# jing2li/MGPreconditionedGCR

Measured on AMD Instinct MI355X. Metric: gcr_iterations_per_sec, higher is better.
Workload: dtype f64; 1 GPU; 3D 7-point Poisson 128^3 per GPU, unpreconditioned GCR restart 5, complex fp64, x0=0, RHS splitmix64 seed 0; rows=2097152, nnz=14581760, complex=True, stored_matrix_bytes=2097292, ell_width=7, tail_nnz=0, partition=1 GPU

## Files before the change

mgpreconditionedgcr_amd/csrc/api.hip:

```cpp
#include <algorithm>
#include <numeric>

#include <cstring>

#include "internal.h"

using namespace mgcr;

#define LOCK() std::lock_guard<std::recursive_mutex> lk__(ctx().mtx)

extern "C" {

int mgcr_csr_create(int64_t nrow, int64_t ncol, const int64_t *rowptr, const int64_t *col, const double *val_ri,
                    mgcr_op_t *out) {
    MGCR_TRY(require_ctx());
    MGCR_CHECK(out && rowptr && (col || rowptr[nrow] == 0) && (val_ri || rowptr[nrow] == 0), MGCR_ERR_INVALID,
               "mgcr_csr_create: null argument");
    LOCK();
    mgcr_op_s *op = new mgcr_op_s();
    op->kind = OP_CSR;
    op->dim = ncol;
    op->nrow = nrow;
    int rc = csr_build_device(nrow, ncol, rowptr, col, val_ri, &op->csr);
    if (rc != MGCR_OK) { delete op; return rc; }
// ... 191 lines not shown

int mgcr_op_halo_kind(mgcr_op_t op, int32_t *kind) {
    MGCR_CHECK(op && kind, MGCR_ERR_INVALID, "mgcr_op_halo_kind: null argument");
    MGCR_REFUSE_EVENODD_MULTI(op, "mgcr_op_halo_kind");
    MGCR_REFUSE_GCR32(op, "mgcr_op_halo_kind");
    const Op *o = op_matrix(op);
    MGCR_CHECK(o->dist, MGCR_ERR_UNSUPPORTED, "mgcr_op_halo_kind: not a distributed Sparse");
    *kind = dist_halo_kind(o->dist);
    return MGCR_OK;
}

int mgcr_set_option(const char *name, int value, int *previous) {
    MGCR_CHECK(name, MGCR_ERR_INVALID, "null option name");
    if (!strcmp(name, "spmv_part")) {
        const int p = set_spmv_part(value);
        if (previous) *previous = p;
        return MGCR_OK;
    }
    bool prev;
    if (!strcmp(name, "pattern_storage")) prev = set_patterns_enabled(value != 0);
    else if (!strcmp(name, "stencil_storage")) prev = set_stencil_enabled(value != 0);
    else if (!strcmp(name, "lean_cycles")) prev = set_lean_enabled(value != 0);
    else if (!strcmp(name, "fused_apply")) prev = set_fuse_enabled(value != 0);
    else if (!strcmp(name, "graph_replay")) prev = set_graph_enabled(value != 0);
    else if (!strcmp(name, "resident_solver")) prev = set_resident_enabled(value != 0);
    else if (!strcmp(name, "step_build")) prev = set_stepbuild_enabled(value != 0);
    else if (!strcmp(name, "start_build")) prev = set_start_build_enabled(value != 0);
    else if (!strcmp(name, "step_build_keep_r")) {
        static bool last = true;
        prev = last;
        last = value != 0;
    }
    else if (!strcmp(name, "step_build_keep_all")) prev = set_stepbuild_keep_all_enabled(value != 0);
    else if (!strcmp(name, "halo_split")) prev = set_halo_split(value != 0);
    else if (!strcmp(name, "pw_tail")) prev = set_pw_tail_enabled(value != 0);
    else { set_error("mgcr_set_option: unknown option '%s'", name); return MGCR_ERR_INVALID; }
    if (previous) *previous = prev ? 1 : 0;
    return MGCR_OK;
}

int mgcr_stat(const char *name, int64_t *value) {
    MGCR_CHECK(name && value, MGCR_ERR_INVALID, "mgcr_stat: null argument");
    if (!strcmp(name, "resident_solves")) *value = resident_solve_count();
    else if (!strcmp(name, "step_build_launches")) *value = stepbuild_launch_count();
    else if (!strcmp(name, "step_keep_wide_launches")) *value = stepbuild_keep_wide_launch_count();
    else if (!strcmp(name, "step_apply_own_launches")) *value = stepbuild_apply_own_launch_count();
    else if (!strcmp(name, "start_build_launches")) *value = start_build_launch_count();
    else if (!strcmp(name, "small_solves")) *value = gcr_small_solve_count();
    else if (!strcmp(name, "one_launch_fallbacks")) *value = gcr_fallback_count();
    else if (!strcmp(name, "halo_split_exchanges")) *value = dist_halo_split_count();
    else if (!strcmp(name, "pw_tail_folds")) *value = comm_pw_tail_count();
    else if (!strcmp(name, "multi_solves")) *value = gcr_multi_solve_count();
    else if (!strcmp(name, "queue_solves")) *value = gcr_queue_stat(0);
    else if (!strcmp(name, "queue_admissions")) *value = gcr_queue_stat(1);
    else if (!strcmp(name, "queue_steps")) *value = gcr_queue_stat(2);
    else if (!strcmp(name, "eo_queue_solves")) *value = gcr_queue_stat(3);
    else if (!strcmp(name, "eo_queue_admissions")) *value = gcr_queue_stat(4);
    else if (!strcmp(name, "eo_queue_steps")) *value = gcr_queue_stat(5);
    else if (!strcmp(name, "evenodd_fused_steps")) *value = eo_fused_step_count();
    else if (!strcmp(name, "evenodd_diag_fused_steps")) *value = eo_diag_fused_step_count();
    else if (!strcmp(name, "evenodd_block_applies")) *value = eo_block_apply_count();
    else if (!strcmp(name, "evenodd_block_fused_steps")) *value = eo_block_fused_step_count();
    else if (!strcmp(name, "gcr32_applies")) *value = gcr32_apply_count();
    else if (!strcmp(name, "gcr32_steps")) *value = gcr32_step_count();
    else { set_error("mgcr_stat: unknown counter '%s'", name); return MGCR_ERR_INVALID; }
    return MGCR_OK;
}

int mgcr_selftest_coherence(int32_t steps, int32_t coherent, int64_t *rows_wrong) {
    MGCR_TRY(require_ctx());
    LOCK();
    return coherence_selftest(steps, coherent, rows_wrong);
}

int mgcr_op_stored_bytes(mgcr_op_t op, int64_t *matrix_bytes, int32_t *ell_width, int64_t *tail_nnz) {
    MGCR_CHECK(op, MGCR_ERR_INVALID, "null operator");
    MGCR_REFUSE_EVENODD_MULTI(op, "mgcr_op_stored_bytes");
    MGCR_REFUSE_GCR32(op, "mgcr_op_stored_bytes");
    const Op *o = op_matrix(op);
// ... 283 lines not shown
```

mgpreconditionedgcr_amd/csrc/gcr_stepbuild.hip:

```cpp
#include <climits>
#include <cstdlib>
#include <type_traits>

#include "internal.h"
#include "reduce.h"
#include "gcr_dev.h"
#include "spmv_dev.h"
#include "exchange_dev.h"

namespace mgcr {

constexpr int SB_MAX_TRIPS = 4;
constexpr int SB_MAX_ND = 5;
constexpr int SB_KEEP_TB = 2;
#ifndef MGCR_SB_KEEP_MORE
#define MGCR_SB_KEEP_MORE 1
#endif
template <bool WIDE, int NDT, bool XR, bool CLOSE, bool REALC> constexpr int sb_kept_rows() {
    if (NDT == 1) return 3;
    if (!REALC || !MGCR_SB_KEEP_MORE) return WIDE ? 0 : 2;
    if (!WIDE) return !XR && CLOSE ? 4 : 3;
    if (NDT == 4) return CLOSE ? 4 : 1;
    return XR ? 2 : 3;
}
#ifndef MGCR_SB_TEMPORAL_TAIL
#define MGCR_SB_TEMPORAL_TAIL -1
#endif
template <bool WIDE, int NDT, bool XR, bool CLOSE, bool REALC> constexpr bool sb_temporal_tail() {
    if (MGCR_SB_TEMPORAL_TAIL >= 0) return MGCR_SB_TEMPORAL_TAIL != 0;
    return REALC && XR && (WIDE ? (NDT == 4 && !CLOSE) || (NDT == 5 && CLOSE) : NDT == 1 && !CLOSE);
}
template <int TB_, int KT_, bool OTF_, int APPLY_, bool TAIL_> struct SbKeepPolicy {
    static constexpr int TB = TB_, KT = KT_;
    static constexpr bool OTF = OTF_, TAIL = TAIL_;
    static constexpr bool OWN = APPLY_ >= 1, LANES = APPLY_ >= 2;
};
#ifndef MGCR_SB_APPLY
#define MGCR_SB_APPLY 1
#endif
template <bool WIDE, int NDT, bool XR, bool CLOSE, bool REALC> constexpr int sb_apply_form() { return REALC ? MGCR_SB_APPLY : 0; }
template <int NDT, bool XR, bool CLOSE> constexpr bool sb_close_merged() { return CLOSE && (NDT == 4 || (NDT == 5 && XR)); }

struct StepBuildArgs {
    RowMat m;
    const cplx *x;
    const cplx *aps[SB_MAX_ND];
    int64_t n;
    int nlogical;
    RowMap rm;
    DevState *st;
    int it;
    const double *partsR;
    int nblkR, strideR;
    double *hist;
    int hist_cap;
    const cplx *den;
    cplx *ap_out;
    double *partsA;
    LeanCoef *lc;
    const cplx *ps[SB_MAX_ND];
    cplx *p_out;
    cplx *xvec;
    cplx *xr_out;
    cplx *xr_den_slot;
    int xr_slot;
    double *partsR_out;
    v4i *slots;
    unsigned gen0;
    unsigned *abort_dev;
    int *abort_host;
    int spin_limit;
    int test_stall;
};

__device__ __forceinline__ cplx sb_xr_alpha(const ResSync &sy, DevState *st, LeanCoef *lc, cplx *xr_den_slot, int xr_slot, int lb) {
    const cplx num = make_double2(res_total(sy, 0), res_total(sy, 1)), den = make_double2(res_total(sy, 2), res_total(sy, 3));
    const cplx alpha = to_sgpr(cdiv(num, den));
    if (lb == 0 && threadIdx.x == 0) {
        *xr_den_slot = den;
        st->npend = xr_slot + 1;
    }
    if (lb == 0 && (int)threadIdx.x < LND) lean_pending_update(lc, xr_slot, alpha, (int)threadIdx.x);
    return alpha;
}

template <int MODE, int WT, int NDT, bool XR, bool CLOSE, bool REALC = false>
__global__ void __launch_bounds__(RED_THREADS, 8) step_build_kernel(StepBuildArgs a) {
    __shared__ double lds[(2 * NDT > 4 ? 2 * NDT : 4) * 17];
    __shared__ double lds_pw[2 * SB_MAX_ND * 17], lds_ws[2 * SB_MAX_ND * RES_GRP];
    __shared__ int gave_up;
    __shared__ cplx sbeta[NDT], scp[NDT];
    extern __shared__ __attribute__((aligned(16))) unsigned char sb_smem[];
    if (a.st->stop_at < a.st->base + a.it) return;
    const int lb = logical_workgroup(a.rm, (int)blockIdx.x, (int)gridDim.x);
    if (lb >= a.nlogical) return;
    cplx *arL = reinterpret_cast<cplx *>(sb_smem);
    ResSync sy;
    res_sync_init(sy, a.slots, a.gen0, a.nlogical, lb, a.abort_dev, a.spin_limit, lds_pw, lds_ws, &gave_up);
    if (a.test_stall && lb == a.test_stall - 1) return;
    int64_t i0, end, stride;
    row_range(a.rm, lb, a.nlogical, a.n, &i0, &end, &stride);
    {
        double v[2 * NDT];
#pragma unroll
        for (int j = 0; j < 2 * NDT; j++) v[j] = 0.;
        int trip = 0;
        for (int64_t i = i0; i < end; i += stride, trip++) {
            const PatLds pl{nullptr, nullptr, nullptr};
            cplx sum;
            if constexpr (REALC) sum = sten_row_product_t<WT, false, 1>(a.m, i, [&](int32_t j) -> cplx { return a.x[j]; });
            else sum = fused_row_product<MODE, WT>(a.m, i, 0, pl, [&](int32_t j) -> cplx { return a.x[j]; });
            const cplx yi = a.m.shift ? csub(a.x[i], cmul(a.m.k, sum)) : sum;
            arL[trip * RED_THREADS + (int)threadIdx.x] = yi;
            __builtin_amdgcn_sched_barrier(0);
            cplx b[NDT];
#pragma unroll
            for (int j = 0; j < NDT; j++) b[j] = ld_stream<true>(a.aps[j] + i);
// ... 124 lines not shown
    if (threadIdx.x < 4) a.partsA[threadIdx.x * RED_MAX_BLOCKS + lb] = mine;
    auto close_last = [&]() {
        if (trip > 0) {
            const int64_t il = i0 + (int64_t)(trip - 1) * stride;
            close_row(il, a.x[il]);
        }
        __builtin_amdgcn_sched_barrier(0);
    };
    if constexpr (XR) {
        if ((int)threadIdx.x < 4) {
            const v4i w4 = {__double2loint(mine), __double2hiint(mine), (int)sy.gen, 0};
            __builtin_amdgcn_raw_buffer_store_b128(w4, sy.slots, ((2 * RES_NV + (int)threadIdx.x) * RES_BLK + lb) * 16, 0, RES_SC1);
        }
        if constexpr (MERGED) close_last();
        const cplx xr0 = i0 < end ? a.x[i0] : make_double2(0., 0.);
        if (!res_collect<4>(sy, 2)) {
            res_abort(a.abort_dev, a.abort_host);
            for (int64_t i = i0; i < end; i += stride) a.xr_out[i] = make_double2(__builtin_nan(""), __builtin_nan(""));
            if (threadIdx.x == 0) a.partsR_out[lb] = __builtin_nan("");
            return;
        }
        if (ends_here) return;
        const cplx alpha = sb_xr_alpha(sy, a.st, a.lc, a.xr_den_slot, a.xr_slot, lb);
        double vr[1] = {0.};
        trip = 0;
        for (int64_t i = i0; i < end; i += stride, trip++) {
            const cplx rn = csub(i == i0 ? xr0 : a.x[i], cmul(alpha, arL[trip * RED_THREADS + (int)threadIdx.x]));
            a.xr_out[i] = rn;
            vr[0] += rn.x * rn.x + rn.y * rn.y;
        }
        const double tot = block_sum_owner<1>(vr, lds);
        if (threadIdx.x == 0) a.partsR_out[lb] = tot;
    }
}

template <class T>
__device__ __forceinline__ T *sb_elem(T *p, uint32_t off) {
    using C = std::conditional_t<std::is_const_v<T>, const char, char>;
    return reinterpret_cast<T *>(reinterpret_cast<C *>(p) + off);
}

__device__ __forceinline__ void sb_wave_pair_to_lds(double (&v)[2], double *lds, int k0) {
    double s;
    const int k = wave_multi_sum<2>(v, s);
    if (((int)threadIdx.x & 31) == 0) lds[(k0 + k) * 17 + ((int)threadIdx.x >> 6)] = s;
}
template <int NV>
__device__ __forceinline__ double sb_block_owner_from_lds(double *lds) {
    const int nwave = (blockDim.x + 63) >> 6;
    __syncthreads();
    double t = 0.;
    if (threadIdx.x < NV)
        for (int w = 0; w < nwave; w++) t += lds[threadIdx.x * 17 + w];
    return t;
}

template <int NDT>
__device__ __forceinline__ const cplx *sb_stage_src(const cplx *den, const LeanCoef *lc, int i) {
    if (i < NDT) return den + i;
    if (i < 2 * NDT) return lc->cx + (i - NDT);
    const int m = (i - 2 * NDT) / NDT, j = (i - 2 * NDT) % NDT;
    return m == 0 ? lc->t + j : lc->T + j * LND + m;
}
template <int NDT>
__device__ __forceinline__ cplx sb_stage_close_coef(const cplx *col, const cplx *sbeta, int m) {
    cplx c = make_double2(0., 0.);
    for (int j = m; j < NDT; j++) c = cadd(c, cmul(sbeta[j], j == m ? make_double2(1., 0.) : col[j]));
    return c;
}
__device__ __forceinline__ void sb_stage_rr_waves(double v, int nblk, double *lds_rr) {
    if (nblk == 1) {
        if (threadIdx.x == 0) lds_rr[16] = v;
        return;
    }
    double w[1] = {v}, s;
    wave_multi_sum<1>(w, s);
    if ((threadIdx.x & 63) == 0) lds_rr[threadIdx.x >> 6] = s;
}
__device__ __forceinline__ double sb_stage_rr(int nblk, const double *lds_rr) {
    if (nblk == 1) return lds_rr[16];
    const int nwave = (blockDim.x + 63) >> 6;
    double t = 0.;
    for (int w = 0; w < nwave; w++) t += lds_rr[w];
    return t;
}

template <int NDT, bool XR, bool CLOSE, bool REALC>
__global__ void __launch_bounds__(RED_THREADS, 8) step_keep_kernel(StepBuildArgs a) {
    using POL = SbKeepPolicy<SB_KEEP_TB, sb_kept_rows<false, NDT, XR, CLOSE, REALC>(), false, sb_apply_form<false, NDT, XR, CLOSE, REALC>(),
                             sb_temporal_tail<false, NDT, XR, CLOSE, REALC>()>;
#include "gcr_stepbuild_keep_body.h"
}
template <int NDT, bool XR, bool CLOSE, bool REALC>
__global__ void __launch_bounds__(RED_THREADS, 8) step_keep_wide_kernel(StepBuildArgs a) {
    using POL = SbKeepPolicy<1, sb_kept_rows<true, NDT, XR, CLOSE, REALC>(), NDT == 5 && XR, sb_apply_form<true, NDT, XR, CLOSE, REALC>(),
                             sb_temporal_tail<true, NDT, XR, CLOSE, REALC>()>;
#include "gcr_stepbuild_keep_body.h"
}

struct StartArgs {
    RowMat m;
    const cplx *b;
    cplx *ap0;
    int64_t n;
    int nlogical;
    RowMap rm;
    DevState *st;
    double *hist;
    LeanCoef *lc;
    cplx *den0;
    cplx *r_out;
    double *partsR_out;
    v4i *slots;
    unsigned gen0;
    unsigned *abort_dev;
    int *abort_host;
    int spin_limit;
// ... 54 lines not shown
        const double nb = res_total(sy, 4);
        a.st->bnorm2 = nb;
        a.st->rr = nb;
        a.hist[0] = sqrt(nb) / sqrt(nb);
    }
    const cplx alpha = sb_xr_alpha(sy, a.st, a.lc, a.den0, 0, lb);
    double vr[1] = {0.};
#pragma unroll
    for (int t = 0; t < SB_MAX_TRIPS; t++) {
        const int64_t i = i0 + (int64_t)t * stride;
        if (i < end) {
            const cplx rn = csub(t == 0 ? b0 : a.b[i], cmul(alpha, apL[t * RED_THREADS + (int)threadIdx.x]));
            a.r_out[i] = rn;
            vr[0] += rn.x * rn.x + rn.y * rn.y;
        }
    }
    const double tot = block_sum_owner<1>(vr, lds);
    if (threadIdx.x == 0) a.partsR_out[lb] = tot;
}

static EnvSwitch g_stepbuild{"MGCR_STEPBUILD"}, g_start_build{"MGCR_START_BUILD"};
static EnvSwitch g_sb_keep_all{"MGCR_SB_KEEP_ALL"};
static EnvSwitch g_sb_real{"MGCR_SB_REAL"};
bool stepbuild_is_enabled() { return g_stepbuild.on(); }
bool set_stepbuild_enabled(bool on) { return g_stepbuild.set(on); }
bool set_start_build_enabled(bool on) { return g_start_build.set(on); }
bool set_stepbuild_keep_all_enabled(bool on) { return g_sb_keep_all.set(on); }
static int64_t g_stepbuild_launches = 0;
int64_t stepbuild_launch_count() { return g_stepbuild_launches; }
static int64_t g_keep_wide_launches = 0;
int64_t stepbuild_keep_wide_launch_count() { return g_keep_wide_launches; }
static int64_t g_apply_own_launches = 0;
int64_t stepbuild_apply_own_launch_count() { return g_apply_own_launches; }

template <int NDT, bool XR, bool CLOSE> constexpr bool sb_keep_fits() { return NDT <= 2 || (NDT == 3 && !(XR && CLOSE)); }
template <int NDT, bool XR, bool CLOSE, bool R> const void *sb_keep(int *form) {
    *form = sb_apply_form<false, NDT, XR, CLOSE, R>();
    if constexpr (sb_keep_fits<NDT, XR, CLOSE>()) return (const void *)step_keep_kernel<NDT, XR, CLOSE, R>;
    else return nullptr;
}
template <int NDT, bool XR, bool CLOSE> constexpr bool sb_keep_wide_fits() { return (NDT == 4 && XR) || (NDT == 5 && CLOSE); }
template <int NDT, bool XR, bool CLOSE, bool R> const void *sb_keep_wide_form(int *form) {
    *form = sb_apply_form<true, NDT, XR, CLOSE, R>();
    if constexpr (sb_keep_wide_fits<NDT, XR, CLOSE>()) return (const void *)step_keep_wide_kernel<NDT, XR, CLOSE, R>;
    else return nullptr;
}
static const void *sb_keep_wide(int nd, bool xr, bool close, bool realc, int *form) {
#define SKR(NDT, R) (close ? (xr ? sb_keep_wide_form<NDT, true, true, R>(form) : sb_keep_wide_form<NDT, false, true, R>(form)) \
                           : (xr ? sb_keep_wide_form<NDT, true, false, R>(form) : sb_keep_wide_form<NDT, false, false, R>(form)))
#define SKK(NDT) (realc ? SKR(NDT, true) : SKR(NDT, false))
    return nd == 4 ? SKK(4) : nd == 5 ? SKK(5) : nullptr;
#undef SKK
#undef SKR
}
static const void *sb_kernel(int nd, bool xr, bool close, bool realc, bool mid, bool *wide = nullptr, bool *own = nullptr) {
    if (wide) *wide = false;
    if (own) *own = false;
    const void *keep = nullptr;
    int form = 0;
    if (g_sb_keep_all.on() && nd > 3) keep = sb_keep_wide(nd, xr, close, realc, &form);
    if (g_sb_keep_all.on() && nd <= 3) {
#define SKR(NDT, R) (close ? (xr ? sb_keep<NDT, true, true, R>(&form) : sb_keep<NDT, false, true, R>(&form)) \
                           : (xr ? sb_keep<NDT, true, false, R>(&form) : sb_keep<NDT, false, false, R>(&form)))
#define SKK(NDT) (realc ? SKR(NDT, true) : SKR(NDT, false))
        keep = nd == 1 ? SKK(1) : nd == 2 ? SKK(2) : SKK(3);
#undef SKK
// ... 66 lines not shown
    a.rm = rm;
    a.st = st;
    a.slots = sh.slots; a.abort_dev = sh.abort_dev; a.abort_host = sh.abort_host;
    a.gen0 = exchange_take_generations(ngen);
    a.test_stall = getenv("MGCR_TEST_STEPBUILD_STALL") ? atoi(getenv("MGCR_TEST_STEPBUILD_STALL")) : 0;
    a.spin_limit = getenv("MGCR_TEST_RESIDENT_SPIN_LIMIT") ? atoi(getenv("MGCR_TEST_RESIDENT_SPIN_LIMIT")) : RES_SPIN_LIMIT;
    return MGCR_OK;
}
static int sb_launch(const void *kernel, void *args, int grid, size_t lds_bytes, const char *who) {
    MGCR_CHECK(launch_is_coresident(kernel, RED_THREADS, lds_bytes, grid), MGCR_ERR_INVALID, "%s: launch would not be co-resident", who);
    void *kargs[1] = {args};
    MGCR_HIP(hipLaunchKernel(kernel, dim3((unsigned)grid), dim3(RED_THREADS), kargs, lds_bytes, ctx().stream));
    MGCR_HIP(hipGetLastError());
    return MGCR_OK;
}

int csr_step_build(const CsrDev &A, const cplx *x, bool shift, cplx k, const cplx *const *aps, int nd, DevState *st, int it, const double *partsR,
                   int nblkR, int strideR, double *hist, int hist_cap, const cplx *den, cplx *ap_out, double *partsA, LeanCoef *lc,
                   const RowMap &rm, cplx *xr_out, cplx *xr_den_slot, int xr_slot, double *partsR_out, const cplx *const *close_ps, cplx *close_p_out,
                   cplx *close_x) {
    MGCR_CHECK(nd >= 1 && nd <= SB_MAX_ND, MGCR_ERR_INVALID, "csr_step_build: 1..5 directions");
    StepBuildArgs a;
    MGCR_TRY(sb_fill_common(a, A, shift, k, st, rm, 3));
    a.x = x;
    for (int j = 0; j < SB_MAX_ND; j++) a.aps[j] = aps[j < nd ? j : 0];
    a.it = it; a.partsR = partsR; a.nblkR = nblkR; a.strideR = strideR; a.hist = hist; a.hist_cap = hist_cap;
    a.den = den; a.ap_out = ap_out; a.partsA = partsA; a.lc = lc;
    for (int j = 0; j < SB_MAX_ND; j++) a.ps[j] = close_ps ? close_ps[j < nd ? j : 0] : nullptr;
    a.p_out = close_p_out; a.xvec = close_x;
    a.xr_out = xr_out; a.xr_den_slot = xr_den_slot; a.xr_slot = xr_slot; a.partsR_out = partsR_out;
    const bool xr = xr_out != nullptr, close = close_ps != nullptr, realc = g_sb_real.on() && a.m.realv;
    bool wide, own;
    const void *kernel = sb_kernel(nd, xr, close, realc, sten_lane_middle(A), &wide, &own);
    MGCR_TRY(sb_launch(kernel, &a, a.nlogical, sb_lds_bytes(A, a.nlogical), "csr_step_build"));
    g_stepbuild_launches++;
    if (wide) g_keep_wide_launches++;
    if (own) g_apply_own_launches++;
    return MGCR_OK;
}

static int64_t g_start_build_launches = 0;
int64_t start_build_launch_count() { return g_start_build_launches; }
static const void *start_kernel(bool realc) {
    return realc ? (const void *)start_build_kernel<true> : (const void *)start_build_kernel<false>;
}

bool csr_start_build_eligible(const CsrDev &A, const DistCsr *dist) {
    if (!g_start_build.on() || !csr_step_build_eligible(A, dist, 1)) return false;
    const bool realc = g_sb_real.on() && row_mat(A, false, cplx{0., 0.}).realv;
    return launch_is_coresident(start_kernel(realc), RED_THREADS, sb_lds_bytes(A, red_grid(A.nrow)), red_grid(A.nrow));
}

int csr_start_build(const CsrDev &A, const cplx *b, bool shift, cplx k, cplx *ap0, DevState *st, double *hist, LeanCoef *lc, cplx *den0,
                    cplx *r_out, double *partsR_out, const RowMap &rm) {
    StartArgs a;
    MGCR_TRY(sb_fill_common(a, A, shift, k, st, rm, 1));
    a.b = b;
    a.ap0 = ap0;
    a.hist = hist; a.lc = lc; a.den0 = den0; a.r_out = r_out; a.partsR_out = partsR_out;
    MGCR_TRY(sb_launch(start_kernel(g_sb_real.on() && a.m.realv), &a, a.nlogical, sb_lds_bytes(A, a.nlogical), "csr_start_build"));
    g_start_build_launches++;
    return MGCR_OK;
}

}
```

mgpreconditionedgcr_amd/csrc/internal.h:

```cpp
#pragma once
#include <hip/hip_runtime.h>
#include <climits>
#include <cstdint>
#include <cstdio>
#include <cstdlib>
#include <cstring>
#include <mutex>
#include <string>
#include <type_traits>
#include <utility>
#include <vector>

#include "../../include/mgcr.h"

namespace mgcr {

typedef double2 cplx;

void set_error(const char *fmt, ...);
int hip_fail(hipError_t e, const char *what, const char *file, int line);

#define MGCR_HIP(call)                                                     \
    do {                                                                   \
        hipError_t e__ = (call);                                           \
// ... 204 lines not shown
template <typename F>
static int dispatch_bool(bool b, F &&f) { return b ? f(std::true_type{}) : f(std::false_type{}); }
template <typename... KA, typename... AA>
static int launch(void (*kernel)(KA...), unsigned grid, int block, size_t lds, AA... args) {
    hipLaunchKernelGGL(kernel, dim3(grid), dim3(block), lds, ctx().stream, args...);
    MGCR_HIP(hipGetLastError());
    return MGCR_OK;
}

int csr_build_device(int64_t nrow, int64_t ncol, const int64_t *h_rowptr, const int64_t *h_col,
                     const double *h_val_ri, CsrDev *out);
void csr_free(CsrDev *c);
bool set_patterns_enabled(bool on);
bool set_stencil_enabled(bool on);
bool stencil_enabled();
int ell_band_count(const CsrDev &A, unsigned long long *d_cnt);
bool csr_stencil_active(const CsrDev &A);
int set_spmv_part(int part);
bool set_lean_enabled(bool on);
bool set_fuse_enabled(bool on);
bool set_graph_enabled(bool on);
bool set_resident_enabled(bool on);
constexpr int MGCR_INT_GAVE_UP = 1001;
int resident_check(bool internal = false);
void resident_shutdown();
int64_t resident_solve_count();
bool set_stepbuild_enabled(bool on);
int64_t stepbuild_launch_count();
int64_t stepbuild_keep_wide_launch_count();
int64_t stepbuild_apply_own_launch_count();
bool set_start_build_enabled(bool on);
int64_t start_build_launch_count();
bool set_stepbuild_keep_all_enabled(bool on);
int coherence_selftest(int steps, int coherent, int64_t *rows_wrong);
bool stepbuild_is_enabled();
bool launch_is_coresident(const void *kernel, int threads, size_t dyn_lds, int grid);
bool one_launch_paths_enabled();
int csr_apply(const CsrDev &A, const cplx *x, cplx *y, bool shift, cplx k, DistCsr *dist = nullptr, const cplx *w = nullptr);
bool csr_fusable(const CsrDev &A, const DistCsr *dist);
bool fuse_enabled();
struct RowMap;
struct PwTail;
bool csr_step_apply_has_pw_tail(const CsrDev &A, const DistCsr *dist);
int csr_step_apply(const CsrDev &A, const cplx *x, cplx *y, bool shift, cplx k, const cplx *const *vecs, int nd, double *parts,
                   DistCsr *dist, const RowMap &rm, const PwTail *pw = nullptr);
struct DevState;
struct LeanCoef;
bool csr_xr_fusable(const CsrDev &A, const DistCsr *dist);
bool csr_apply_carry(const CsrDev &A, const cplx *x, cplx *y, bool shift, cplx k, const cplx *w);
int csr_xr_fuse_kind(const CsrDev &A, const DistCsr *dist);
int csr_step_apply_xr(const CsrDev &A, const cplx *r_in, const cplx *ap, cplx *r_out, cplx *y, bool shift, cplx k, const cplx *const *vecs,
                      int nd, double *parts, double *partsR, DevState *st, int it, const double *partsA, int nblkA, int strideA,
                      cplx *den_slot, int slot, LeanCoef *lc, const RowMap &rm);
int csr_init_apply(const CsrDev &A, const cplx *r0, cplx *aps0, bool shift, cplx k, const cplx *b, double *partsA, double *partsR,
                   double *partsN, DistCsr *dist, const RowMap &rm);
int bcsr_build_device(int32_t nbrow, int32_t nbcol, int32_t bs, const int32_t *h_browptr, const int32_t *h_bcol,
                      const double *h_blocks, BcsrDev *out);
void bcsr_free(BcsrDev *b);
int bcsr_apply(const BcsrDev &A, const cplx *x, cplx *y, const cplx *xh = nullptr, int32_t nb_own = INT32_MAX);

struct SkipRef {
    const int *p = nullptr;
    int it = 0;
};
void set_apply_skip(SkipRef s);
SkipRef get_apply_skip();
// ... 121 lines not shown
```

Measured before the change: 16200 it/s.

## Add paired-workgroup step-build kernel merging two logical blocks per CTA

Adds a new step_pair_kernel in which each physical workgroup handles two logical workgroups, launched on half the grid (256 instead of 512) when the logical grid is 512 and the kernel can be co-resident. Each thread keeps more rows of Ap_0/Ap_1 in registers, and one combined poll/collect serves both logical blocks. The aim is to cut the cost of grid-wide synchronisation and to reuse more data held on chip in the fused GCR step. The cost is higher register pressure (launch bounds lowered to 4) and fewer resident waves. It applies only to realc, xr, non-shifted forms with keep_all on, and is gated by the MGCR_SB_PAIR env switch, whose default is not visible.

Result: faster. 16860 it/s (median of 6 runs) (+4.0%).

```diff
diff --git a/mgpreconditionedgcr_amd/csrc/api.hip b/mgpreconditionedgcr_amd/csrc/api.hip
--- a/mgpreconditionedgcr_amd/csrc/api.hip
+++ b/mgpreconditionedgcr_amd/csrc/api.hip
@@ -247,6 +247,7 @@
         last = value != 0;
     }
     else if (!strcmp(name, "step_build_keep_all")) prev = set_stepbuild_keep_all_enabled(value != 0);
+    else if (!strcmp(name, "step_build_pair")) prev = set_stepbuild_pair_enabled(value != 0);
     else if (!strcmp(name, "halo_split")) prev = set_halo_split(value != 0);
     else if (!strcmp(name, "pw_tail")) prev = set_pw_tail_enabled(value != 0);
     else { set_error("mgcr_set_option: unknown option '%s'", name); return MGCR_ERR_INVALID; }
@@ -260,6 +261,7 @@
     else if (!strcmp(name, "step_build_launches")) *value = stepbuild_launch_count();
     else if (!strcmp(name, "step_keep_wide_launches")) *value = stepbuild_keep_wide_launch_count();
     else if (!strcmp(name, "step_apply_own_launches")) *value = stepbuild_apply_own_launch_count();
+    else if (!strcmp(name, "step_pair_launches")) *value = stepbuild_pair_launch_count();
     else if (!strcmp(name, "start_build_launches")) *value = start_build_launch_count();
     else if (!strcmp(name, "small_solves")) *value = gcr_small_solve_count();
     else if (!strcmp(name, "one_launch_fallbacks")) *value = gcr_fallback_count();
diff --git a/mgpreconditionedgcr_amd/csrc/gcr_stepbuild.hip b/mgpreconditionedgcr_amd/csrc/gcr_stepbuild.hip
--- a/mgpreconditionedgcr_amd/csrc/gcr_stepbuild.hip
+++ b/mgpreconditionedgcr_amd/csrc/gcr_stepbuild.hip
@@ -7,11 +7,10 @@
 #include "gcr_dev.h"
 #include "spmv_dev.h"
 #include "exchange_dev.h"
+#include "gcr_stepbuild_dev.h"
 
 namespace mgcr {
 
-constexpr int SB_MAX_TRIPS = 4;
-constexpr int SB_MAX_ND = 5;
 constexpr int SB_KEEP_TB = 2;
 #ifndef MGCR_SB_KEEP_MORE
 #define MGCR_SB_KEEP_MORE 1
@@ -40,49 +39,6 @@
 #endif
 template <bool WIDE, int NDT, bool XR, bool CLOSE, bool REALC> constexpr int sb_apply_form() { return REALC ? MGCR_SB_APPLY : 0; }
 template <int NDT, bool XR, bool CLOSE> constexpr bool sb_close_merged() { return CLOSE && (NDT == 4 || (NDT == 5 && XR)); }
-
-struct StepBuildArgs {
-    RowMat m;
-    const cplx *x;
-    const cplx *aps[SB_MAX_ND];
-    int64_t n;
-    int nlogical;
-    RowMap rm;
-    DevState *st;
-    int it;
-    const double *partsR;
-    int nblkR, strideR;
-    double *hist;
-    int hist_cap;
-    const cplx *den;
-    cplx *ap_out;
-    double *partsA;
-    LeanCoef *lc;
-    const cplx *ps[SB_MAX_ND];
-    cplx *p_out;
-    cplx *xvec;
-    cplx *xr_out;
-    cplx *xr_den_slot;
-    int xr_slot;
-    double *partsR_out;
-    v4i *slots;
-    unsigned gen0;
-    unsigned *abort_dev;
-    int *abort_host;
-    int spin_limit;
-    int test_stall;
-};
-
-__device__ __forceinline__ cplx sb_xr_alpha(const ResSync &sy, DevState *st, LeanCoef *lc, cplx *xr_den_slot, int xr_slot, int lb) {
-    const cplx num = make_double2(res_total(sy, 0), res_total(sy, 1)), den = make_double2(res_total(sy, 2), res_total(sy, 3));
-    const cplx alpha = to_sgpr(cdiv(num, den));
-    if (lb == 0 && threadIdx.x == 0) {
-        *xr_den_slot = den;
-        st->npend = xr_slot + 1;
-    }
-    if (lb == 0 && (int)threadIdx.x < LND) lean_pending_update(lc, xr_slot, alpha, (int)threadIdx.x);
-    return alpha;
-}
 
 template <int MODE, int WT, int NDT, bool XR, bool CLOSE, bool REALC = false>
 __global__ void __launch_bounds__(RED_THREADS, 8) step_build_kernel(StepBuildArgs a) {
@@ -273,57 +229,6 @@
         const double tot = block_sum_owner<1>(vr, lds);
         if (threadIdx.x == 0) a.partsR_out[lb] = tot;
     }
-}
-
-template <class T>
-__device__ __forceinline__ T *sb_elem(T *p, uint32_t off) {
-    using C = std::conditional_t<std::is_const_v<T>, const char, char>;
-    return reinterpret_cast<T *>(reinterpret_cast<C *>(p) + off);
-}
-
-__device__ __forceinline__ void sb_wave_pair_to_lds(double (&v)[2], double *lds, int k0) {
-    double s;
-    const int k = wave_multi_sum<2>(v, s);
-    if (((int)threadIdx.x & 31) == 0) lds[(k0 + k) * 17 + ((int)threadIdx.x >> 6)] = s;
-}
-template <int NV>
-__device__ __forceinline__ double sb_block_owner_from_lds(double *lds) {
-    const int nwave = (blockDim.x + 63) >> 6;
-    __syncthreads();
-    double t = 0.;
-    if (threadIdx.x < NV)
-        for (int w = 0; w < nwave; w++) t += lds[threadIdx.x * 17 + w];
-    return t;
-}
-
-template <int NDT>
-__device__ __forceinline__ const cplx *sb_stage_src(const cplx *den, const LeanCoef *lc, int i) {
-    if (i < NDT) return den + i;
-    if (i < 2 * NDT) return lc->cx + (i - NDT);
-    const int m = (i - 2 * NDT) / NDT, j = (i - 2 * NDT) % NDT;
-    return m == 0 ? lc->t + j : lc->T + j * LND + m;
-}
-template <int NDT>
-__device__ __forceinline__ cplx sb_stage_close_coef(const cplx *col, const cplx *sbeta, int m) {
-    cplx c = make_double2(0., 0.);
-    for (int j = m; j < NDT; j++) c = cadd(c, cmul(sbeta[j], j == m ? make_double2(1., 0.) : col[j]));
-    return c;
-}
-__device__ __forceinline__ void sb_stage_rr_waves(double v, int nblk, double *lds_rr) {
-    if (nblk == 1) {
-        if (threadIdx.x == 0) lds_rr[16] = v;
-        return;
-    }
-    double w[1] = {v}, s;
-    wave_multi_sum<1>(w, s);
-    if ((threadIdx.x & 63) == 0) lds_rr[threadIdx.x >> 6] = s;
-}
-__device__ __forceinline__ double sb_stage_rr(int nblk, const double *lds_rr) {
-    if (nblk == 1) return lds_rr[16];
-    const int nwave = (blockDim.x + 63) >> 6;
-    double t = 0.;
-    for (int w = 0; w < nwave; w++) t += lds_rr[w];
-    return t;
 }
 
 template <int NDT, bool XR, bool CLOSE, bool REALC>
@@ -444,6 +349,8 @@
 int64_t stepbuild_keep_wide_launch_count() { return g_keep_wide_launches; }
 static int64_t g_apply_own_launches = 0;
 int64_t stepbuild_apply_own_launch_count() { return g_apply_own_launches; }
+static int64_t g_pair_launches = 0;
+int64_t stepbuild_pair_launch_count() { return g_pair_launches; }
 
 template <int NDT, bool XR, bool CLOSE> constexpr bool sb_keep_fits() { return NDT <= 2 || (NDT == 3 && !(XR && CLOSE)); }
 template <int NDT, bool XR, bool CLOSE, bool R> const void *sb_keep(int *form) {
@@ -576,7 +483,14 @@
     const bool xr = xr_out != nullptr, close = close_ps != nullptr, realc = g_sb_real.on() && a.m.realv;
     bool wide, own;
     const void *kernel = sb_kernel(nd, xr, close, realc, sten_lane_middle(A), &wide, &own);
-    MGCR_TRY(sb_launch(kernel, &a, a.nlogical, sb_lds_bytes(A, a.nlogical), "csr_step_build"));
+    const void *pair = own && !shift && g_sb_keep_all.on() && a.nlogical == SB_PAIR_LOGICAL && exchange_shared().cus >= SB_PAIR_GRID
+                           ? sb_pair_kernel(nd, xr, close, realc) : nullptr;
+    if (pair && launch_is_coresident(pair, RED_THREADS, SB_PAIR_LDS, SB_PAIR_GRID)) {
+        MGCR_TRY(sb_launch(pair, &a, SB_PAIR_GRID, SB_PAIR_LDS, "csr_step_build (pair form)"));
+        g_pair_launches++;
+    } else {
+        MGCR_TRY(sb_launch(kernel, &a, a.nlogical, sb_lds_bytes(A, a.nlogical), "csr_step_build"));
+    }
     g_stepbuild_launches++;
     if (wide) g_keep_wide_launches++;
     if (own) g_apply_own_launches++;
diff --git a/mgpreconditionedgcr_amd/csrc/gcr_stepbuild_dev.h b/mgpreconditionedgcr_amd/csrc/gcr_stepbuild_dev.h
--- /dev/null
+++ b/mgpreconditionedgcr_amd/csrc/gcr_stepbuild_dev.h
@@ -0,0 +1,112 @@
+#pragma once
+#include <type_traits>
+
+#include "internal.h"
+#include "reduce.h"
+#include "gcr_dev.h"
+#include "exchange_dev.h"
+
+namespace mgcr {
+
+constexpr int SB_MAX_TRIPS = 4;
+constexpr int SB_MAX_ND = 5;
+
+struct StepBuildArgs {
+    RowMat m;
+    const cplx *x;
+    const cplx *aps[SB_MAX_ND];
+    int64_t n;
+    int nlogical;
+    RowMap rm;
+    DevState *st;
+    int it;
+    const double *partsR;
+    int nblkR, strideR;
+    double *hist;
+    int hist_cap;
+    const cplx *den;
+    cplx *ap_out;
+    double *partsA;
+    LeanCoef *lc;
+    const cplx *ps[SB_MAX_ND];
+    cplx *p_out;
+    cplx *xvec;
+    cplx *xr_out;
+    cplx *xr_den_slot;
+    int xr_slot;
+    double *partsR_out;
+    v4i *slots;
+    unsigned gen0;
+    unsigned *abort_dev;
+    int *abort_host;
+    int spin_limit;
+    int test_stall;
+};
+
+__device__ __forceinline__ cplx sb_xr_alpha(const ResSync &sy, DevState *st, LeanCoef *lc, cplx *xr_den_slot, int xr_slot, int lb) {
+    const cplx num = make_double2(res_total(sy, 0), res_total(sy, 1)), den = make_double2(res_total(sy, 2), res_total(sy, 3));
+    const cplx alpha = to_sgpr(cdiv(num, den));
+    if (lb == 0 && threadIdx.x == 0) {
+        *xr_den_slot = den;
+        st->npend = xr_slot + 1;
+    }
+    if (lb == 0 && (int)threadIdx.x < LND) lean_pending_update(lc, xr_slot, alpha, (int)threadIdx.x);
+    return alpha;
+}
+
+template <class T>
+__device__ __forceinline__ T *sb_elem(T *p, uint32_t off) {
+    using C = std::conditional_t<std::is_const_v<T>, const char, char>;
+    return reinterpret_cast<T *>(reinterpret_cast<C *>(p) + off);
+}
+
+__device__ __forceinline__ void sb_wave_pair_to_lds(double (&v)[2], double *lds, int k0) {
+    double s;
+    const int k = wave_multi_sum<2>(v, s);
+    if (((int)threadIdx.x & 31) == 0) lds[(k0 + k) * 17 + ((int)threadIdx.x >> 6)] = s;
+}
+template <int NV>
+__device__ __forceinline__ double sb_block_owner_from_lds(double *lds) {
+    const int nwave = (blockDim.x + 63) >> 6;
+    __syncthreads();
+    double t = 0.;
+    if (threadIdx.x < NV)
+        for (int w = 0; w < nwave; w++) t += lds[threadIdx.x * 17 + w];
+    return t;
+}
+
+template <int NDT>
+__device__ __forceinline__ const cplx *sb_stage_src(const cplx *den, const LeanCoef *lc, int i) {
+    if (i < NDT) return den + i;
+    if (i < 2 * NDT) return lc->cx + (i - NDT);
+    const int m = (i - 2 * NDT) / NDT, j = (i - 2 * NDT) % NDT;
+    return m == 0 ? lc->t + j : lc->T + j * LND + m;
+}
+template <int NDT>
+__device__ __forceinline__ cplx sb_stage_close_coef(const cplx *col, const cplx *sbeta, int m) {
+    cplx c = make_double2(0., 0.);
+    for (int j = m; j < NDT; j++) c = cadd(c, cmul(sbeta[j], j == m ? make_double2(1., 0.) : col[j]));
+    return c;
+}
+__device__ __forceinline__ void sb_stage_rr_waves(double v, int nblk, double *lds_rr) {
+    if (nblk == 1) {
+        if (threadIdx.x == 0) lds_rr[16] = v;
+        return;
+    }
+    double w[1] = {v}, s;
+    wave_multi_sum<1>(w, s);
+    if ((threadIdx.x & 63) == 0) lds_rr[threadIdx.x >> 6] = s;
+}
+__device__ __forceinline__ double sb_stage_rr(int nblk, const double *lds_rr) {
+    if (nblk == 1) return lds_rr[16];
+    const int nwave = (blockDim.x + 63) >> 6;
+    double t = 0.;
+    for (int w = 0; w < nwave; w++) t += lds_rr[w];
+    return t;
+}
+
+const void *sb_pair_kernel(int nd, bool xr, bool close, bool realc);
+constexpr size_t SB_PAIR_LDS = sizeof(cplx) * RED_THREADS * 2 * SB_MAX_TRIPS;
+constexpr int SB_PAIR_LOGICAL = 512, SB_PAIR_GRID = SB_PAIR_LOGICAL / 2;
+
+}
diff --git a/mgpreconditionedgcr_amd/csrc/gcr_steppair.hip b/mgpreconditionedgcr_amd/csrc/gcr_steppair.hip
--- /dev/null
+++ b/mgpreconditionedgcr_amd/csrc/gcr_steppair.hip
@@ -0,0 +1,335 @@
+#include "internal.h"
+#include "reduce.h"
+#include "gcr_dev.h"
+#include "spmv_dev.h"
+#include "exchange_dev.h"
+#include "gcr_stepbuild_dev.h"
+
+namespace mgcr {
+
+constexpr int SP_ROWS = 2 * SB_MAX_TRIPS;
+#ifndef MGCR_SB_PAIR_KEPT
+#define MGCR_SB_PAIR_KEPT -1
+#endif
+template <int NDT, bool CLOSE> constexpr int sb_pair_kept() {
+    if (NDT == 1) return SP_ROWS;
+    if (MGCR_SB_PAIR_KEPT >= 0) return MGCR_SB_PAIR_KEPT;
+    return NDT == 2 ? 15 : NDT == 3 ? 14 : NDT == 4 ? 11 : 12;
+}
+#ifndef MGCR_SB_PAIR_P1
+#define MGCR_SB_PAIR_P1 8
+#endif
+#ifndef MGCR_SB_PAIR_TB
+#define MGCR_SB_PAIR_TB 2
+#endif
+#ifndef MGCR_SB_PAIR_XR_STREAM
+#define MGCR_SB_PAIR_XR_STREAM 0
+#endif
+#ifndef MGCR_SB_PAIR_FORMS
+#define MGCR_SB_PAIR_FORMS -1
+#endif
+template <int NDT, bool XR, bool CLOSE> constexpr bool sb_pair_built() { return XR && (CLOSE ? NDT == 5 : NDT <= 4); }
+template <int NDT, bool XR, bool CLOSE> constexpr bool sb_pair_form() {
+    if (!sb_pair_built<NDT, XR, CLOSE>()) return false;
+    if (MGCR_SB_PAIR_FORMS >= 0) return MGCR_SB_PAIR_FORMS != 0;
+    return !CLOSE && NDT >= 2;
+}
+
+template <int H, int LN>
+__device__ __forceinline__ void sp_wave_sums_to_lds(double (&v)[2 * H], double (&lds)[2][LN], int k0) {
+    static_assert(H == 1 || H == 2 || H == 4, "2 H scalars: a power of two, every lane group owns one");
+    double s;
+    const int k = wave_multi_sum<2 * H>(v, s);
+    if (((int)threadIdx.x & (64 / (2 * H) - 1)) == 0) lds[k / H][(k0 + k % H) * 17 + ((int)threadIdx.x >> 6)] = s;
+}
+template <int NV, int LN>
+__device__ __forceinline__ double sp_block_owner_from_lds(const double (&lds)[2][LN]) {
+    __syncthreads();
+    const int w = (int)threadIdx.x >> 6, k = (int)threadIdx.x & 63;
+    double t = 0.;
+    if (w < 2 && k < NV)
+        for (int q = 0; q < RED_THREADS / 64; q++) t += lds[w][k * 17 + q];
+    return t;
+}
+
+__device__ __forceinline__ double sp_poll(ResSync &s, int at, unsigned want) {
+    int spins = 0;
+    for (;;) {
+        const v4i w = __builtin_amdgcn_raw_buffer_load_b128(s.slots, at, 0, RES_SC1);
+        if ((unsigned)w.z == want) return __hiloint2double(w.y, w.x);
+        spins++;
+        if (spins > s.spin_limit || ((spins & 255) == 0 && __hip_atomic_load(s.abort_dev, __ATOMIC_RELAXED, __HIP_MEMORY_SCOPE_AGENT) != 0u)) {
+            *s.gave_up = 1;
+            return 0.;
+        }
+        __builtin_amdgcn_s_sleep(1);
+    }
+}
+template <int NVT>
+__device__ __forceinline__ bool sp_collect(ResSync &s, int kind, const int (&lbs)[2]) {
+    static_assert(NVT <= RES_NV, "scalars per exchange");
+    const int lane = threadIdx.x & 63, wave = threadIdx.x >> 6;
+    const int ng = (s.nblk + 63) >> 6;
+    for (int task = (wave >> 1) * s.nblk + lbs[wave & 1]; task < ng * NVT; task += (RED_THREADS / 128) * s.nblk) {
+        const int g = task / NVT, k = task - g * NVT;
+        const int blk = g * 64 + lane;
+        const double v = blk < s.nblk ? sp_poll(s, ((kind * RES_NV + k) * RES_BLK + blk) * 16, s.gen) : 0.;
+        double t = wave_sum(v);
+        t = __shfl(t, 0, 64);
+        if (lane < RES_COPIES) {
+            const v4i w4 = {__double2loint(t), __double2hiint(t), (int)s.gen, 0};
+            __builtin_amdgcn_raw_buffer_store_b128(w4, s.slots, RES_L2_BASE + ((lane * 3 + kind) * RES_NV + k) * RES_GRP * 16 + g * 16, 0, RES_SC1);
+        }
+    }
+    if ((int)threadIdx.x < RES_GRP * NVT) {
+        const int k = (int)threadIdx.x / RES_GRP, g = (int)threadIdx.x % RES_GRP;
+        const int copy = s.lb & (RES_COPIES - 1);
+        s.ws[k * RES_GRP + g] = g < ng ? sp_poll(s, RES_L2_BASE + ((copy * 3 + kind) * RES_NV + k) * RES_GRP * 16 + g * 16, s.gen) : 0.;
+    }
+    __syncthreads();
+    s.gen++;
+    return *s.gave_up == 0;
+}
+
+template <int NDT, bool CLOSE>
+__global__ void __launch_bounds__(RED_THREADS, 4) step_pair_kernel(StepBuildArgs a) {
+    constexpr int KT = sb_pair_kept<NDT, CLOSE>();
+    constexpr int K0 = KT < SP_ROWS ? KT : SP_ROWS, K1 = NDT >= 2 && KT > SP_ROWS ? KT - SP_ROWS : 0;
+    static_assert(KT >= 0 && KT <= 2 * SP_ROWS, "rows of Ap_0 and Ap_1");
+    constexpr int P1 = MGCR_SB_PAIR_P1, TB = MGCR_SB_PAIR_TB;
+    static_assert(SP_ROWS % P1 == 0 && SP_ROWS % TB == 0, "whole batches");
+    constexpr int SB_STAGE_N = CLOSE ? 2 * NDT + NDT * NDT : NDT;
+    constexpr int LN = (2 * NDT > 4 ? 2 * NDT : 4) * 17;
+    __shared__ double lds[2][LN];
+    __shared__ double lds_pw[2 * SB_MAX_ND * 17], lds_ws[2 * SB_MAX_ND * RES_GRP];
+    __shared__ int gave_up;
+    __shared__ cplx sbeta[NDT], scp[NDT];
+    __shared__ double lds_rr[17];
+    __shared__ cplx sstg[SB_STAGE_N];
+    extern __shared__ __attribute__((aligned(16))) unsigned char sb_smem[];
+    if (a.st->stop_at < a.st->base + a.it) return;
+    const int p1 = (((int)blockIdx.x >> 3) << 4) | ((int)blockIdx.x & 7);
+    const int lbs[2] = {logical_workgroup(a.rm, p1, a.nlogical), logical_workgroup(a.rm, p1 + 8, a.nlogical)};
+    if (lbs[0] >= a.nlogical || lbs[1] >= a.nlogical) return;
+    const bool has0 = lbs[0] == 0 || lbs[1] == 0;
+    cplx *arL = reinterpret_cast<cplx *>(sb_smem);
+    const int tid = (int)threadIdx.x;
+    const int own_w = tid >> 6, own_k = tid & 63;
+    const int own_lb = lbs[own_w & 1];
+    ResSync sy;
+    res_sync_init(sy, a.slots, a.gen0, a.nlogical, lbs[0], a.abort_dev, a.spin_limit, lds_pw, lds_ws, &gave_up);
+    if (a.test_stall && (lbs[0] == a.test_stall - 1 || lbs[1] == a.test_stall - 1)) return;
+    int64_t i0[2], end[2], stride, stride_b;
+    row_range(a.rm, lbs[0], a.nlogical, a.n, &i0[0], &end[0], &stride);
+    row_range(a.rm, lbs[1], a.nlogical, a.n, &i0[1], &end[1], &stride_b);
+    auto row = [&](int u) -> int64_t { return i0[u / SB_MAX_TRIPS] + (int64_t)(u % SB_MAX_TRIPS) * stride; };
+    auto live = [&](int u) -> bool { return row(u) < end[u / SB_MAX_TRIPS]; };
+    uint32_t off[SP_ROWS];
+#pragma unroll
+    for (int u = 0; u < SP_ROWS; u++) off[u] = (uint32_t)row(u) * (uint32_t)sizeof(cplx);
+    auto at = [&](auto *p, int u) { return sb_elem(p, off[u]); };
+    cplx rk[SP_ROWS];
+#pragma unroll
+    for (int u = 0; u < SP_ROWS; u++) {
+        const int64_t i = row(u), e = end[u / SB_MAX_TRIPS];
+        rk[u] = make_double2(0., 0.);
+        const auto xj = [&](int32_t j) -> cplx { return *sb_elem(a.x, (uint32_t)j * (uint32_t)sizeof(cplx)); };
+        if (__builtin_amdgcn_readfirstlane((int32_t)i) < (int32_t)e) {
+            cplx own;
+            const cplx sum = sten_row_product_own_t<1, false>(a.m, i, xj, own);
+            if (i < e) {
+                rk[u] = own;
+                arL[u * RED_THREADS + tid] = sum;
+            }
+        }
+        __builtin_amdgcn_sched_barrier(0);
+    }
+    {
+        const double stg_r = a.nblkR == 1 ? (tid == 0 ? a.partsR[0] + 0. : 0.) : (tid < a.nblkR ? a.partsR[tid] : 0.);
+        cplx stg_c = make_double2(0., 0.);
+        const int stg_i = tid - (RED_THREADS - 64);
+        if (stg_i >= 0 && stg_i < SB_STAGE_N) stg_c = *sb_stage_src<NDT>(a.den, a.lc, stg_i);
+        sb_stage_rr_waves(stg_r, a.nblkR, lds_rr);
+        if (stg_i >= 0 && stg_i < SB_STAGE_N) sstg[stg_i] = stg_c;
+    }
+    __builtin_amdgcn_sched_barrier(0);
+    cplx pre0[K0 > 0 ? K0 : 1], pre1[K1 > 0 ? K1 : 1];
+    {
+#pragma unroll
+        for (int jj = 0; jj < NDT; jj++) {
+            const int j = NDT - 1 - jj;
+            double v[4] = {0., 0., 0., 0.};
+#pragma unroll
+            for (int u0 = 0; u0 < SP_ROWS; u0 += P1) {
+                cplx b[P1];
+#pragma unroll
+                for (int q = 0; q < P1; q++) b[q] = live(u0 + q) ? ld_stream<true>(at(a.aps[j], u0 + q)) : make_double2(0., 0.);
+#pragma unroll
+                for (int q = 0; q < P1; q++) {
+                    const int u = u0 + q;
+                    if (live(u)) {
+                        const cplx tt = cconj_mul(arL[u * RED_THREADS + tid], b[q]);
+                        v[2 * (u / SB_MAX_TRIPS)] += tt.x;
+                        v[2 * (u / SB_MAX_TRIPS) + 1] += tt.y;
+                    }
+                    if (j == 0 && u < K0) pre0[u < K0 ? u : 0] = b[q];
+                    if (j == 1 && u < K1) pre1[u < K1 ? u : 0] = b[q];
+                }
+                if (P1 < SP_ROWS) __builtin_amdgcn_sched_barrier(0);
+            }
+            sp_wave_sums_to_lds<2>(v, lds, 2 * j);
+            __builtin_amdgcn_sched_barrier(0);
+        }
+        const double mine = sp_block_owner_from_lds<2 * NDT>(lds);
+        if (own_w < 2 && own_k < 2 * NDT) {
+            const v4i w4 = {__double2loint(mine), __double2hiint(mine), (int)sy.gen, 0};
+            __builtin_amdgcn_raw_buffer_store_b128(w4, sy.slots, ((1 * RES_NV + own_k) * RES_BLK + own_lb) * 16, 0, RES_SC1);
+        }
+    }
+    const bool ends_here = __builtin_amdgcn_readfirstlane(!((sb_stage_rr(a.nblkR, lds_rr) / a.st->bnorm2) > a.st->tol2)) != 0;
+    if (!sp_collect<2 * NDT>(sy, 1, lbs)) {
+        res_abort(a.abort_dev, a.abort_host);
+#pragma unroll
+        for (int u = 0; u < SP_ROWS; u++)
+            if (live(u)) *at(a.ap_out, u) = make_double2(__builtin_nan(""), __builtin_nan(""));
+        if (own_w < 2 && own_k < 4) a.partsA[own_k * RED_MAX_BLOCKS + own_lb] = __builtin_nan("");
+        return;
+    }
+    if (has0 && tid == 0) {
+        close_step(a.st, a.it, sb_stage_rr(a.nblkR, lds_rr), a.hist, a.hist_cap, CLOSE);
+        if (CLOSE) a.st->closed = 1;
+    }
+    if (tid < NDT) sbeta[tid] = cdiv(make_double2(res_total(sy, 2 * tid), res_total(sy, 2 * tid + 1)), sstg[tid]);
+    __syncthreads();
+    if constexpr (CLOSE) {
+        if (tid < NDT) scp[tid] = sb_stage_close_coef<NDT>(sstg + 2 * NDT + tid * NDT, sbeta, tid);
+        __syncthreads();
+    }
+    if (!CLOSE && has0 && tid <= NDT) lean_table_row<NDT>(a.lc, sbeta, tid);
+    {
+        cplx beta[NDT];
+#pragma unroll
+        for (int j = 0; j < NDT; j++) beta[j] = to_sgpr(sbeta[j]);
+        double v[8] = {0., 0., 0., 0., 0., 0., 0., 0.};
+#pragma unroll
+        for (int u0 = 0; u0 < SP_ROWS; u0 += TB) {
+            cplx ac[TB];
+#pragma unroll
+            for (int q = 0; q < TB; q++) ac[q] = make_double2(0., 0.);
+#pragma unroll
+            for (int j = 0; j < NDT; j++) {
+                cplx aj[TB];
+#pragma unroll
+                for (int q = 0; q < TB; q++) {
+                    const int u = u0 + q;
+                    aj[q] = (j == 0 && u < K0)   ? pre0[u < K0 ? u : 0]
+                            : (j == 1 && u < K1) ? pre1[u < K1 ? u : 0]
+                            : live(u)            ? ld_stream<NTS>(at(a.aps[j], u))
+                                                 : make_double2(0., 0.);
+                }
+#pragma unroll
+                for (int q = 0; q < TB; q++) ac[q] = csub(ac[q], cmul(beta[j], aj[q]));
+                __builtin_amdgcn_sched_barrier(0);
+            }
+#pragma unroll
+            for (int q = 0; q < TB; q++) {
+                const int u = u0 + q, h = 4 * (u / SB_MAX_TRIPS);
+                if (live(u)) {
+                    const cplx an = cadd(arL[u * RED_THREADS + tid], ac[q]);
+                    *at(a.ap_out, u) = an;
+                    arL[u * RED_THREADS + tid] = an;
+                    const cplx tt = cconj_mul(rk[u], an);
+                    v[h] += tt.x; v[h + 1] += tt.y;
+                    const cplx w = cconj_mul(an, an);
+                    v[h + 2] += w.x; v[h + 3] += w.y;
+                }
+            }
+        }
+        sp_wave_sums_to_lds<4>(v, lds, 0);
+        const double mine = sp_block_owner_from_lds<4>(lds);
+        if (own_w < 2 && own_k < 4) {
+            a.partsA[own_k * RED_MAX_BLOCKS + own_lb] = mine;
+            const v4i w4 = {__double2loint(mine), __double2hiint(mine), (int)sy.gen, 0};
+            __builtin_amdgcn_raw_buffer_store_b128(w4, sy.slots, ((2 * RES_NV + own_k) * RES_BLK + own_lb) * 16, 0, RES_SC1);
+        }
+    }
+    if constexpr (CLOSE) {
+        cplx cx[NDT], cp[NDT];
+#pragma unroll
+        for (int j = 0; j < NDT; j++) {
+            cx[j] = to_sgpr(sstg[NDT + j]);
+            cp[j] = to_sgpr(scp[j]);
+        }
+#pragma unroll
+        for (int u0 = 0; u0 < SP_ROWS; u0 += TB) {
+            cplx xv[TB], pc[TB];
+#pragma unroll
+            for (int q = 0; q < TB; q++) {
+                xv[q] = live(u0 + q) ? *at(a.xvec, u0 + q) : make_double2(0., 0.);
+                pc[q] = make_double2(0., 0.);
+            }
+#pragma unroll
+            for (int j = 0; j < NDT; j++) {
+                cplx pj[TB];
+#pragma unroll
+                for (int q = 0; q < TB; q++) pj[q] = live(u0 + q) ? ld_stream<NTS>(at(a.ps[j], u0 + q)) : make_double2(0., 0.);
+#pragma unroll
+                for (int q = 0; q < TB; q++) {
+                    xv[q] = cadd(xv[q], cmul(cx[j], pj[q]));
+                    pc[q] = csub(pc[q], cmul(cp[j], pj[q]));
+                }
+            }
+#pragma unroll
+            for (int q = 0; q < TB; q++) {
+                if (live(u0 + q)) {
+                    *at(a.xvec, u0 + q) = xv[q];
+                    st_stream<NTS>(at(a.p_out, u0 + q), cadd(rk[u0 + q], pc[q]));
+                }
+            }
+            __builtin_amdgcn_sched_barrier(0);
+        }
+    }
+    if (!sp_collect<4>(sy, 2, lbs)) {
+        res_abort(a.abort_dev, a.abort_host);
+#pragma unroll
+        for (int u = 0; u < SP_ROWS; u++)
+            if (live(u)) *at(a.xr_out, u) = make_double2(__builtin_nan(""), __builtin_nan(""));
+        if (own_w < 2 && own_k == 0) a.partsR_out[own_lb] = __builtin_nan("");
+        return;
+    }
+    if (ends_here) return;
+    const cplx alpha = sb_xr_alpha(sy, a.st, a.lc, a.xr_den_slot, a.xr_slot, has0 ? 0 : 1);
+    double vr[2] = {0., 0.};
+#pragma unroll
+    for (int u = 0; u < SP_ROWS; u++) {
+        if (live(u)) {
+            const cplx rn = csub(rk[u], cmul(alpha, arL[u * RED_THREADS + tid]));
+            st_stream<MGCR_SB_PAIR_XR_STREAM != 0>(at(a.xr_out, u), rn);
+            vr[u / SB_MAX_TRIPS] += rn.x * rn.x + rn.y * rn.y;
+        }
+    }
+    sp_wave_sums_to_lds<1>(vr, lds, 0);
+    const double tot = sp_block_owner_from_lds<1>(lds);
+    if (own_w < 2 && own_k == 0) a.partsR_out[own_lb] = tot;
+}
+
+static EnvSwitch g_sb_pair{"MGCR_SB_PAIR"};
+bool set_stepbuild_pair_enabled(bool on) { return g_sb_pair.set(on); }
+
+template <int NDT, bool XR, bool CLOSE> static const void *sb_pair_entry() {
+    if constexpr (sb_pair_form<NDT, XR, CLOSE>()) return (const void *)step_pair_kernel<NDT, CLOSE>;
+    else return nullptr;
+}
+const void *sb_pair_kernel(int nd, bool xr, bool close, bool realc) {
+    if (!g_sb_pair.on() || !realc || !xr) return nullptr;
+    if (close) return nd == 5 ? sb_pair_entry<5, true, true>() : nullptr;
+    switch (nd) {
+        case 1: return sb_pair_entry<1, true, false>();
+        case 2: return sb_pair_entry<2, true, false>();
+        case 3: return sb_pair_entry<3, true, false>();
+        case 4: return sb_pair_entry<4, true, false>();
+        default: return nullptr;
+    }
+}
+
+}
diff --git a/mgpreconditionedgcr_amd/csrc/internal.h b/mgpreconditionedgcr_amd/csrc/internal.h
--- a/mgpreconditionedgcr_amd/csrc/internal.h
+++ b/mgpreconditionedgcr_amd/csrc/internal.h
@@ -260,6 +260,8 @@
 bool set_start_build_enabled(bool on);
 int64_t start_build_launch_count();
 bool set_stepbuild_keep_all_enabled(bool on);
+bool set_stepbuild_pair_enabled(bool on);
+int64_t stepbuild_pair_launch_count();
 int coherence_selftest(int steps, int coherent, int64_t *rows_wrong);
 bool stepbuild_is_enabled();
 bool launch_is_coresident(const void *kernel, int threads, size_t dyn_lds, int grid);
```
